# zhengfei0908/SBA-GAN

Hardware: AMD Instinct MI355X
Metric: images/sec (G+D step) at 256px (higher is better)
Workload: dtype bf16; 1 GPU; bird_style.yml 3-stage G+D step (64..256px), B=20 per GPU, G_NET variant=model, image_encoder=inception, text_encoder=RNN_ENCODER in the step; global_batch=20, parallelism=dp1, launch=replayer, losses_finite=True

## Files before the change

include/sbagan_hip.h:

```cpp
#ifndef SBAGAN_HIP_H
#define SBAGAN_HIP_H

#include <stdint.h>

#ifdef __cplusplus
extern "C" {
#endif

#define SBA_F32 0
#define SBA_BF16 1
#define SBA_BF16_YH 2

#define SBA_OK 0
#define SBA_E_ARG (-1)
#define SBA_E_LAUNCH (-2)
#define SBA_E_UNSUPPORTED (-3)

#define SBA_ACT_NONE 0
#define SBA_ACT_GLU 1
#define SBA_ACT_LRELU 2
#define SBA_ACT_RELU 3

#define SBA_MAX_TAPS 32

typedef struct sba_conv_geom {
    int32_t N, IH, IW, Cin;
    int32_t OH, OW, Cout;
    int32_t OHs, OWs;
    int32_t sy, sx;
    int32_t osy, osx, ooy, oox;
    int32_t ups;
    int32_t ntaps;
    int8_t ty[SBA_MAX_TAPS];
    int8_t tx[SBA_MAX_TAPS];
    int32_t x_cstride, x_coff, y_cstride, y_coff;
    int32_t relu;
    int32_t tile, ksplit;
    int32_t first_write;
    int32_t w_layout;
} sba_conv_geom;
#define SBA_IGEMM_TILES 18

const char* sba_version(void);

int sba_set_deterministic(int on, void* scratch, int64_t scratch_bytes);
int sba_get_deterministic(void);
int sba_det_reset(void);
int64_t sba_det_high_water(void);
int sba_set_reduce_scratch(void* scratch, int64_t scratch_bytes);
int sba_bn_stat_slots(void);

int sba_conv_igemm(int dtype, const void* x, const void* w, void* y, const void* addend,
                   float* stats, const sba_conv_geom* g, void* workspace, int64_t workspace_bytes,
                   void* stream);
int sba_conv_igemm_bias(int dtype, const void* x, const void* w, void* y, const void* addend,
                        float* stats, const float* bias, const void* relu_mask, const sba_conv_geom* g,
                        void* workspace, int64_t workspace_bytes, void* stream);
int sba_conv_igemm_plan(int dtype, const sba_conv_geom* g, int64_t workspace_bytes, int* plan);

int sba_fold_bn_pack(int dtype, const float* w, const float* gamma, const float* beta, const float* running_mean,
                     const float* running_var, float eps, void* out, float* bias, int O, int taps, int Cin, int glu,
                     void* stream);
int sba_conv_igemm_glu(int dtype, const void* x, const void* w, const float* bias, void* y, int C,
                       const sba_conv_geom* g, void* stream);
int sba_conv_igemm_glu_plan(int dtype, const sba_conv_geom* g, int C, int* plan);
#define SBA_GROUP_MAX 8
typedef struct sba_conv_group_item {
    const void* x; const void* w; void* y; const void* addend; const float* bias; const void* relu_mask;
    const sba_conv_geom* g;
} sba_conv_group_item;
int sba_conv_igemm_group(int dtype, int n, const sba_conv_group_item* items, int tile, void* stream);
int sba_conv_igemm_group_splitk(int dtype, int n, const sba_conv_group_item* items, int tile, int ksplit,
// ... 216 lines not shown
```

sba-gan_amd/csrc/igemm.hip:

```cpp
#include <math.h>
#include <stdlib.h>

#include "common.h"
#include <type_traits>

namespace {

struct FastDiv {
    uint64_t magic;
    uint32_t d;
};
static inline FastDiv make_fastdiv(uint32_t d, int64_t max_n) {
    FastDiv f;
    f.d = d;
    f.magic = (max_n < (1 << 21) && d > 0) ? (((uint64_t)1 << 42) + d - 1) / d : 0;
    return f;
}
__device__ __forceinline__ uint32_t fdiv(uint32_t n, const FastDiv& f) {
    return f.magic ? (uint32_t)(((uint64_t)n * f.magic) >> 42) : n / f.d;
}

struct EpiX { const float* bias; const void* mask; int yh; int glu_c; };

__device__ __forceinline__ uint32_t relu_mask_bf16x2(uint32_t v, uint32_t m) {
// ... 25 lines not shown
            for (int j = 0; j < TN; ++j)
                b[j] = *reinterpret_cast<const bf16x8_t*>(b_rows + (j * 32 + r) * ROWB + kk * 32 + h * 16);
#pragma unroll
            for (int i = 0; i < TM; ++i)
#pragma unroll
                for (int j = 0; j < TN; ++j)
                    acc[i][j] = __builtin_amdgcn_mfma_f32_32x32x16_bf16(a[i], b[j], acc[i][j], 0, 0, 0);
        }
    }
};

template <> struct Mma<float> {
    template <int TM, int TN, int ROWB>
    static __device__ __forceinline__ void slab(const unsigned char* a_rows, const unsigned char* b_rows,
                                                int lane, f32x16_t (&acc)[TM][TN]) {
        const int r = lane & 31, h = lane >> 5;
#pragma unroll
        for (int kk = 0; kk < 8; ++kk) {
            float a[TM], b[TN];
#pragma unroll
            for (int i = 0; i < TM; ++i)
                a[i] = *reinterpret_cast<const float*>(a_rows + (i * 32 + r) * ROWB + (2 * kk + h) * 4);
#pragma unroll
            for (int j = 0; j < TN; ++j)
                b[j] = *reinterpret_cast<const float*>(b_rows + (j * 32 + r) * ROWB + (2 * kk + h) * 4);
#pragma unroll
            for (int i = 0; i < TM; ++i)
#pragma unroll
                for (int j = 0; j < TN; ++j)
                    acc[i][j] = __builtin_amdgcn_mfma_f32_32x32x2f32(a[i], b[j], acc[i][j], 0, 0, 0);
        }
    }
};

template <typename T, int BM, int BN, int TM, int TN, int NTT, int STAGE_BYTES>
__device__ __forceinline__ void tile_epilogue(f32x16_t (&acc)[TM][TN], const bool lead, unsigned char* lds_all,
                                              const int* rowoff, float* s_stat, const int wm0, const int wn0,
                                              const int lane, const int n_base, const int ycs,
                                              const sba_conv_geom& g, T* __restrict__ y,
                                              const T* __restrict__ addend, float* __restrict__ stats,
                                              const EpiX ex, const int slot_id = -1) {
    const float* __restrict__ bias = ex.bias;
    const T* __restrict__ rmask = reinterpret_cast<const T*>(ex.mask);
    const int col_l = lane & 31, rsel = 4 * (lane >> 5);
    constexpr bool kStageOut = sizeof(T) == 2;
    constexpr int OROW = BN * 2 + 16;
    static_assert(!kStageOut || BM * OROW <= STAGE_BYTES, "output tile fits in the staging buffers");
    if (lead) {
#pragma unroll
    for (int j = 0; j < TN; ++j) {
        const int co = n_base + wn0 + j * 32 + col_l;
        float csum = 0.f, csq = 0.f;
        const float bco = bias ? bias[co < g.Cout ? co : 0] : 0.f;
#pragma unroll
        for (int i = 0; i < TM; ++i) {
#pragma unroll
            for (int r = 0; r < 16; ++r) {
                const int row = wm0 + i * 32 + (r & 3) + 8 * (r >> 2) + rsel;
                float v = acc[i][j][r];
                csum += v;
                csq += v * v;
                if (bias) v += bco;
                if (g.relu) v = fmaxf(v, 0.f);
                if (kStageOut) {
                    *reinterpret_cast<bf16_t*>(lds_all + row * OROW + (wn0 + j * 32 + col_l) * 2) =
                        ex.yh ? f2h_bits(v) : f2bf(v);
                } else {
                    const int pix = rowoff[row];
                    if (pix >= 0 && co < g.Cout) {
                        const int64_t o = (int64_t)pix * ycs + g.y_coff + co;
                        if (addend) v += to_f<T>(addend[o]);
                        if (rmask && !(to_f<T>(rmask[o]) > 0.f)) v = 0.f;
                        y[o] = from_f<T>(v);
                    }
                }
            }
        }
        if (stats) {
            csum += __shfl_xor(csum, 32, 64);
            csq += __shfl_xor(csq, 32, 64);
            if (lane < 32) {
                atomicAdd(&s_stat[wn0 + j * 32 + col_l], csum);
                atomicAdd(&s_stat[BN + wn0 + j * 32 + col_l], csq);
            }
        }
    }
    }
    if (kStageOut || stats) __syncthreads();
    if (kStageOut) {
        constexpr int CPRO = BN / 8;
        for (int idx = threadIdx.x; idx < BM * CPRO; idx += NTT) {
            const int row = idx / CPRO, cc = idx - row * CPRO;
            const int pix = rowoff[row];
            const int co = n_base + cc * 8;
            if (pix < 0 || co >= g.Cout) continue;
            uint4 v = *reinterpret_cast<const uint4*>(lds_all + row * OROW + cc * 16);
            const int64_t o = (int64_t)pix * ycs + g.y_coff + co;
            if (co + 8 <= g.Cout) {
                if (addend) {
                    const uint4 a = *reinterpret_cast<const uint4*>(addend + o);
                    v.x = add_bf16x2(v.x, a.x);
                    v.y = add_bf16x2(v.y, a.y);
                    v.z = add_bf16x2(v.z, a.z);
                    v.w = add_bf16x2(v.w, a.w);
                }
                if (rmask) {
                    const uint4 m = *reinterpret_cast<const uint4*>(rmask + o);
                    v.x = relu_mask_bf16x2(v.x, m.x);
                    v.y = relu_mask_bf16x2(v.y, m.y);
                    v.z = relu_mask_bf16x2(v.z, m.z);
                    v.w = relu_mask_bf16x2(v.w, m.w);
                }
                *reinterpret_cast<uint4*>(y + o) = v;
            } else {
                const uint32_t vw[4] = {v.x, v.y, v.z, v.w};
#pragma unroll
                for (int k = 0; k < 8; ++k) {
                    if (co + k < g.Cout) {
                        float f = bf2f((bf16_t)((k & 1) ? (vw[k >> 1] >> 16) : (vw[k >> 1] & 0xffffu)));
                        if (addend) f += to_f<T>(addend[o + k]);
                        if (rmask && !(to_f<T>(rmask[o + k]) > 0.f)) f = 0.f;
                        y[o + k] = from_f<T>(f);
                    }
                }
            }
        }
    }
    if (stats) {
        const int sid = slot_id >= 0 ? slot_id : (int)(blockIdx.x + blockIdx.z);
        float* slot = stats + (int64_t)(sid & (SBA_BN_STAT_SLOTS - 1)) * 2 * g.Cout;
        for (int c = threadIdx.x; c < BN; c += NTT) {
            const int co = n_base + c;
            if (co < g.Cout) {
                atomicAdd(&slot[co], s_stat[c]);
                atomicAdd(&slot[g.Cout + co], s_stat[BN + c]);
            }
        }
    }
}

template <typename T, int BM, int BN, int TM, int TN, int NTT, int STAGE_BYTES>
__device__ __forceinline__ void tile_epilogue_glu(f32x16_t (&acc)[TM][TN], unsigned char* lds_all, const int* rowoff,
                                                  const int wm0, const int wn0, const int lane, const int n_base,
                                                  const sba_conv_geom& g, T* __restrict__ y, const EpiX ex) {
    static_assert(TN % 2 == 0 && BN % 64 == 0, "a wave owns whole (value, gate) granule pairs");
    const float* __restrict__ bias = ex.bias;
    const int C = ex.glu_c;
    const int ycs = g.y_cstride ? g.y_cstride : C;
    const int col_l = lane & 31, rsel = 4 * (lane >> 5);
    constexpr bool kStageOut = sizeof(T) == 2;
    constexpr int BNO = BN / 2;
    constexpr int OROW = BNO * 2 + 16;
    static_assert(!kStageOut || BM * OROW <= STAGE_BYTES, "output tile fits in the staging buffers");
#pragma unroll
    for (int j = 0; j < TN; j += 2) {
        const int rv = n_base + wn0 + j * 32 + col_l;
        const float bv = bias[rv], bg = bias[rv + 32];
        const int lc = (wn0 >> 1) + (j >> 1) * 32 + col_l;
        const int oc = (n_base >> 1) + lc;
#pragma unroll
        for (int i = 0; i < TM; ++i) {
// ... 2130 lines not shown
            o.y = (uint32_t)f2bf(tile[c8 + 2][r]) | ((uint32_t)f2bf(tile[c8 + 3][r]) << 16);
            o.z = (uint32_t)f2bf(tile[c8 + 4][r]) | ((uint32_t)f2bf(tile[c8 + 5][r]) << 16);
            o.w = (uint32_t)f2bf(tile[c8 + 6][r]) | ((uint32_t)f2bf(tile[c8 + 7][r]) << 16);
            *reinterpret_cast<uint4*>(op) = o;
        } else {
#pragma unroll
            for (int k = 0; k < 8; ++k)
                if (co + k < d.Cout) op[k] = from_f<T>(tile[c8 + k][r]);
        }
    }
}

template <typename T>
__global__ void pool2x2_kernel(const T* __restrict__ up, T* __restrict__ dx, int N, int H, int W, int C) {
    constexpr int V = Vec16<T>::N;
    const int cv = C / V;
    const int64_t total = (int64_t)N * H * W * cv;
    for (int64_t i = blockIdx.x * (int64_t)blockDim.x + threadIdx.x; i < total;
         i += (int64_t)gridDim.x * blockDim.x) {
        const int c = (int)(i % cv) * V;
        int64_t p = i / cv;
        const int xx = (int)(p % W); p /= W;
        const int yy = (int)(p % H);
        const int n = (int)(p / H);
        const T* b = up + (((int64_t)n * 2 * H + 2 * yy) * 2 * W + 2 * xx) * C + c;
        Vec16<T> v00 = ld16(b), v01 = ld16(b + C), v10 = ld16(b + (int64_t)2 * W * C),
                 v11 = ld16(b + (int64_t)2 * W * C + C), o;
#pragma unroll
        for (int k = 0; k < V; ++k) o.set(k, v00.get(k) + v01.get(k) + v10.get(k) + v11.get(k));
        st16(dx + (((int64_t)n * H + yy) * W + xx) * C + c, o);
    }
}

template <typename T>
__device__ __forceinline__ void splitk_finish_body(float* __restrict__ ws, T* __restrict__ y,
                                                   const T* __restrict__ addend,
                                                   float* __restrict__ stats, const sba_conv_geom& g,
                                                   const int M, const EpiX ex) {
    const int ycs = g.y_cstride ? g.y_cstride : g.Cout;
    const int cq = g.Cout / 4;
    const int t = blockIdx.x * blockDim.x + threadIdx.x;
    if (t >= cq) return;
    const int c = t * 4;
    const int m0 = blockIdx.y * 8, m1 = min(m0 + 8, M);
    if (m0 >= M) return;
    const int sub = g.OHs * g.OWs;
    float s0[4] = {0.f, 0.f, 0.f, 0.f}, s1[4] = {0.f, 0.f, 0.f, 0.f};
    float4 rows[8];
#pragma unroll
    for (int r = 0; r < 8; ++r) {
        const int m = m0 + r;
        float4* wp = reinterpret_cast<float4*>(ws + (int64_t)(m < m1 ? m : m0) * g.Cout + c);
        rows[r] = *wp;
        if (m < m1) *wp = make_float4(0.f, 0.f, 0.f, 0.f);
    }
    float bv[4] = {0.f, 0.f, 0.f, 0.f};
    if (ex.bias) {
#pragma unroll
        for (int k = 0; k < 4; ++k) bv[k] = ex.bias[c + k];
    }
#pragma unroll
    for (int r = 0; r < 8; ++r) {
        const int m = m0 + r;
        if (m >= m1) break;
        float v[4] = {rows[r].x, rows[r].y, rows[r].z, rows[r].w};
        const int n = m / sub, rem = m - n * sub;
        const int oy = rem / g.OWs, ox = rem - oy * g.OWs;
        const int64_t o = ((int64_t)(n * g.OH + oy * g.osy + g.ooy) * g.OW + ox * g.osx + g.oox) * ycs + g.y_coff + c;
        typedef typename std::conditional<sizeof(T) == 2, uint2, uint4>::type V4;
        T av[4], mv[4], ov[4];
        if (addend) *reinterpret_cast<V4*>(av) = *reinterpret_cast<const V4*>(addend + o);
        if (ex.mask) *reinterpret_cast<V4*>(mv) = *reinterpret_cast<const V4*>(reinterpret_cast<const T*>(ex.mask) + o);
#pragma unroll
        for (int k = 0; k < 4; ++k) {
            s0[k] += v[k];
            s1[k] += v[k] * v[k];
            v[k] += bv[k];
            if (g.relu) v[k] = fmaxf(v[k], 0.f);
            if (addend) v[k] += to_f<T>(av[k]);
            if (ex.mask && !(to_f<T>(mv[k]) > 0.f)) v[k] = 0.f;
            if (sizeof(T) == 2 && ex.yh) *reinterpret_cast<bf16_t*>(&ov[k]) = f2h_bits(v[k]);
            else ov[k] = from_f<T>(v[k]);
        }
        *reinterpret_cast<V4*>(y + o) = *reinterpret_cast<const V4*>(ov);
    }
    if (stats) {
        float* slot = stats + (int64_t)(blockIdx.y & (SBA_BN_STAT_SLOTS - 1)) * 2 * g.Cout;
#pragma unroll
        for (int k = 0; k < 4; ++k) {
            atomicAdd(&slot[c + k], s0[k]);
            atomicAdd(&slot[g.Cout + c + k], s1[k]);
        }
    }
}

template <typename T>
__global__ __launch_bounds__(256) void splitk_finish_kernel(float* __restrict__ ws, T* __restrict__ y,
                                                            const T* __restrict__ addend,
                                                            float* __restrict__ stats, const sba_conv_geom g,
                                                            const int M, const EpiX ex) {
    splitk_finish_body<T>(ws, y, addend, stats, g, M, ex);
}

__global__ __launch_bounds__(256) void splitk_finish_group_kernel(const GroupArgs A) {
    const GroupItem& it = A.it[blockIdx.z];
    const sba_conv_geom g = it.g;
    splitk_finish_body<bf16_t>(it.ws, it.y, it.addend, nullptr, g, it.M, EpiX{it.bias, it.mask, 0});
}

struct IgemmCfg { int bm, bn, ks, occ; float eff; bool split; };
static const IgemmCfg kCfg[5] = {
    {128, 128, 1, 3, 1.00f, false}, {256, 64, 1, 3, 1.00f, false}, {128, 64, 2, 2, 0.80f, false},
    {64, 64, 2, 4, 0.50f, true},    {320, 128, 2, 1, 0.90f, true}};
constexpr int IGEMM_SPLIT_MAX_M = 2048;

template <typename T, int BM, int BN, int WM, int WN, int KS>
static void launch_cfg(const T* xp, const T* wp, T* yp, const T* ap, float* stats, const sba_conv_geom& g, int M,
                       int nslabs, int split, float* ws, hipStream_t st, const EpiX ex) {
    constexpr int NT = (BM / WM) * (BN / WN) * 64;
    int sps = nslabs;
    if (split > 1) {
        sps = cdiv(cdiv(nslabs, split), KS) * KS;
        split = cdiv(nslabs, sps);
    }
    dim3 grid(cdiv(M, BM), cdiv(g.Cout, BN), split);
    SBA_LAUNCH((igemm_kernel<T, BM, BN, WM, WN, KS>), grid, dim3(NT), 0, st, xp, wp, yp, ap, stats, g, M,
                       split > 1 ? ws : (float*)nullptr, sps, ex);
    if (split > 1) {
        dim3 fgrid(cdiv(g.Cout / 4, 256), cdiv(M, 8));
        SBA_LAUNCH((splitk_finish_kernel<T>), fgrid, dim3(256), 0, st, ws, yp, ap, stats, g, M, ex);
    }
}

static int nmajor_for(const sba_conv_geom& g) {
    const int64_t wb = (int64_t)g.Cout * g.ntaps * g.Cin, xb = (int64_t)g.N * g.IH * g.IW * g.Cin;
    return wb > xb ? 1 : 0;
}

template <int BM, int BN, int WM, int WN, int KS, int D>
static void launch_dma(const bf16_t* xp, const bf16_t* wp, bf16_t* yp, const bf16_t* ap, float* stats,
                       const sba_conv_geom& g, int M, int nslabs, int split, float* ws, hipStream_t st, const EpiX ex) {
    constexpr int NT = (BM / WM) * (BN / WN) * 64;
    int sps = nslabs;
    if (split > 1) {
        sps = cdiv(cdiv(nslabs, split), KS) * KS;
        split = cdiv(nslabs, sps);
    }
    const int gx = cdiv(M, BM), gy = cdiv(g.Cout, BN);
    const int nmajor = nmajor_for(g);
    dim3 grid(nmajor ? 8 * cdiv(gy, 8) * gx : 8 * cdiv(gx, 8) * gy, 1, split);
    SBA_LAUNCH((igemm_dma_kernel<BM, BN, WM, WN, KS, D>), grid, dim3(NT), 0, st, xp, wp, yp, ap, stats, g, M,
               split > 1 ? ws : (float*)nullptr, sps, ex, gx, gy, nmajor DMA_TRACE_ARG);
    if (split > 1) {
        dim3 fgrid(cdiv(g.Cout / 4, 256), cdiv(M, 8));
        SBA_LAUNCH((splitk_finish_kernel<bf16_t>), fgrid, dim3(256), 0, st, ws, yp, ap, stats, g, M, ex);
    }
}

template <int BM, int BN, int WM, int WN, int D>
static void launch_dma2(const bf16_t* xp, const bf16_t* wp, bf16_t* yp, const bf16_t* ap, float* stats,
                        const sba_conv_geom& g, int M, int nslabs64, int split, float* ws, hipStream_t st, const EpiX ex) {
    constexpr int NT = (BM / WM) * (BN / WN) * 64;
    int sps = nslabs64;
    if (split > 1) {
        sps = cdiv(nslabs64, split);
        split = cdiv(nslabs64, sps);
    }
    const int gx = cdiv(M, BM), gy = cdiv(g.Cout, BN);
    const int nmajor = nmajor_for(g);
    dim3 grid(nmajor ? 8 * cdiv(gy, 8) * gx : 8 * cdiv(gx, 8) * gy, 1, split);
    SBA_LAUNCH((igemm_dma2_kernel<BM, BN, WM, WN, D>), grid, dim3(NT), 0, st, xp, wp, yp, ap, stats, g, M,
               split > 1 ? ws : (float*)nullptr, sps, ex, gx, gy, nmajor DMA_TRACE_ARG);
    if (split > 1) {
        dim3 fgrid(cdiv(g.Cout / 4, 256), cdiv(M, 8));
        SBA_LAUNCH((splitk_finish_kernel<bf16_t>), fgrid, dim3(256), 0, st, ws, yp, ap, stats, g, M, ex);
    }
}

static bool halo_ok(const sba_conv_geom& g) {
    if (g.ntaps != 9 || g.sy != 1 || g.sx != 1 || g.osy != 1 || g.osx != 1 || g.ooy || g.oox) return false;
    if (g.OHs != g.OH || g.OWs != g.OW || (g.Cin != 64 && g.Cin != 128) || g.Cout % 64) return false;
    if (g.OH % 8 || g.OW % 32) return false;
    if (g.ups ? (g.IH * 2 != g.OH || g.IW * 2 != g.OW) : (g.IH != g.OH || g.IW != g.OW)) return false;
    for (int t = 0; t < 9; ++t)
        if (g.ty[t] != t / 3 - 1 || g.tx[t] != t % 3 - 1) return false;
    const int64_t tiles = (int64_t)g.N * (g.OH / 8) * (g.OW / 32);
    return tiles >= 128 && tiles <= 0x7fffffff;
}

static bool halo3g_ok(const sba_conv_geom& g) {
    if (g.w_layout != 1 || g.ups) return false;
    if (g.ntaps != 9 || g.sy != 1 || g.sx != 1 || g.osy != 1 || g.osx != 1 || g.ooy || g.oox) return false;
    if (g.OHs != g.OH || g.OWs != g.OW || g.Cin % 32 || g.Cout % 32) return false;
    int ymin = g.ty[0], ymax = g.ty[0], xmin = g.tx[0], xmax = g.tx[0];
    unsigned seen = 0;
    for (int t = 0; t < 9; ++t) {
        ymin = g.ty[t] < ymin ? g.ty[t] : ymin; ymax = g.ty[t] > ymax ? g.ty[t] : ymax;
        xmin = g.tx[t] < xmin ? g.tx[t] : xmin; xmax = g.tx[t] > xmax ? g.tx[t] : xmax;
    }
    if (ymax - ymin != 2 || xmax - xmin != 2) return false;
    for (int t = 0; t < 9; ++t) seen |= 1u << ((g.ty[t] - ymin) * 3 + (g.tx[t] - xmin));
    if (seen != 0x1ffu) return false;
    const int64_t tiles = (int64_t)g.N * cdiv(g.OH, 8) * cdiv(g.OW, 32);
    return tiles >= 128 && tiles <= 0x7fffffff;
}

static void launch_halo3g(const sba_conv_geom& g, const bf16_t* x, const bf16_t* w, bf16_t* y, const bf16_t* addend,
                          const EpiX ex, hipStream_t st) {
    const int tiles = g.N * cdiv(g.OH, 8) * cdiv(g.OW, 32);
    const bool tn2 = g.Cout % 64 == 0;
    dim3 grid(tiles, g.Cout / (tn2 ? 64 : 32));
    if (g.Cin % 64 == 0) {
        if (tn2) SBA_LAUNCH((conv3x3_halo3g_kernel<64, 2>), grid, dim3(256), 0, st, x, w, y, addend, g, ex);
        else SBA_LAUNCH((conv3x3_halo3g_kernel<64, 1>), grid, dim3(256), 0, st, x, w, y, addend, g, ex);
    } else {
        if (tn2) SBA_LAUNCH((conv3x3_halo3g_kernel<32, 2>), grid, dim3(256), 0, st, x, w, y, addend, g, ex);
        else SBA_LAUNCH((conv3x3_halo3g_kernel<32, 1>), grid, dim3(256), 0, st, x, w, y, addend, g, ex);
    }
}

static void launch_halo(const sba_conv_geom& g, const bf16_t* x, const bf16_t* w, bf16_t* y, const bf16_t* addend,
                        float* stats, const EpiX ex, hipStream_t st) {
    const int tiles = g.N * (g.OH / 8) * (g.OW / 32);
    dim3 grid(tiles, g.Cout / 64);
    if (g.w_layout == 1) {
        if (g.ups) SBA_LAUNCH((conv3x3_halo3_kernel<64, 1>), grid, dim3(256), 0, st, x, w, y, addend, stats, g, ex);
        else SBA_LAUNCH((conv3x3_halo3_kernel<64, 0>), grid, dim3(256), 0, st, x, w, y, addend, stats, g, ex);
        return;
    }
    if (g.ups) SBA_LAUNCH((conv3x3_halo_kernel<64, 64, 1>), grid, dim3(256), 0, st, x, w, y, addend, stats, g, ex);
    else SBA_LAUNCH((conv3x3_halo_kernel<64, 64, 0>), grid, dim3(256), 0, st, x, w, y, addend, stats, g, ex);
}

template <typename T>
int launch_igemm(const void* x, const void* w, void* y, const void* addend, float* stats,
                 const sba_conv_geom& g, void* workspace, int64_t ws_bytes, hipStream_t st,
                 const EpiX ex = EpiX{nullptr, nullptr, 0}, int* plan = nullptr) {
    const int M = g.N * g.OHs * g.OWs;
    const T* xp = (const T*)x; const T* wp = (const T*)w; T* yp = (T*)y; const T* ap = (const T*)addend;
    if (g.w_layout != 0 && !(g.w_layout == 1 && sizeof(T) == 2 && (halo_ok(g) || halo3g_ok(g)))) return SBA_E_ARG;
    if (sizeof(T) == 2 && g.w_layout == 1 && !halo_ok(g)) {
        if (plan) { plan[0] = 4; plan[1] = g.Cin % 64 == 0 ? 64 : 32; plan[2] = 1; return SBA_OK; }
        if (stats) return SBA_E_ARG;
        launch_halo3g(g, (const bf16_t*)x, (const bf16_t*)w, (bf16_t*)y, (const bf16_t*)addend, ex, st);
        return SBA_CHECK_LAUNCH();
    }
    if (sizeof(T) == 2 && halo_ok(g)) {
        if (plan) { plan[0] = 0; plan[1] = g.ups ? 1 : 0; plan[2] = 1; return SBA_OK; }
        launch_halo(g, (const bf16_t*)x, (const bf16_t*)w, (bf16_t*)y, (const bf16_t*)addend, stats, ex, st);
        return SBA_CHECK_LAUNCH();
    }
    const int nslabs = g.ntaps * (g.Cin / (64 / (int)sizeof(T)));
    const bool can_split = workspace && g.Cout % 4 == 0 && (int64_t)M * g.Cout * 4 <= ws_bytes && nslabs >= 16;
    int best, best_split = 1;
    const int wgA = (g.Cout % 128 == 0) ? cdiv(M, 128) * (g.Cout / 128) : 0;
    if (M <= 2048) {
        best = (g.Cout >= 1024 && (nslabs >= 512 || (M >= 1280 && nslabs >= 256))) ? 4 : 3;
    } else if ((g.Cout == 128 && M >= 40000) || (g.Cout == 256 && M >= 40000 && nslabs >= 48)) {
        best = 4;
    } else if (wgA >= 320) {
        best = 0;
    } else if (g.Cout <= 64 && cdiv(M, 256) >= 256) {
        best = 1;
    } else if (cdiv(M, 128) * cdiv(g.Cout, 64) >= 256) {
        best = 2;
    } else {
        best = 3;
    }
    {
        const IgemmCfg& k = kCfg[best];
        const int tiles = cdiv(M, k.bm) * cdiv(g.Cout, k.bn);
        const int slots = 256 * k.occ;
        if (k.split && can_split && tiles < slots && M <= IGEMM_SPLIT_MAX_M) {
            int split = slots / tiles;
            if (split > nslabs / 8) split = nslabs / 8;
            if (split > 32) split = 32;
            if (split > 1) best_split = split;
        }
    }
    const bool det = sba_det_on();
// ... 197 lines not shown
    if (O <= 0 || taps <= 0 || Cin <= 0 || (glu && O % 2)) return SBA_E_ARG;
    const int rows = glu ? 64 * ((O / 2 + 31) / 32) : O;
    const int64_t n = (int64_t)rows * taps * Cin;
    if ((int64_t)taps * Cin > 0x7fffffff) return SBA_E_ARG;
    const int blocks = (int)((n + 255) / 256 > 4096 ? 4096 : (n + 255) / 256);
    SBA_DISPATCH(dtype, SBA_LAUNCH((fold_bn_pack_kernel<T>), dim3(blocks), dim3(256), 0, (hipStream_t)stream, w, gamma,
                                   beta, running_mean, running_var, eps, (T*)out, bias, O, taps * Cin, glu, n));
    return SBA_CHECK_LAUNCH();
}

extern "C" int sba_conv_igemm_glu(int dtype, const void* x, const void* w, const float* bias, void* y, int C,
                                  const sba_conv_geom* g, void* stream) {
    sba_conv_geom gg;
    if (!x || !w || !bias || !y || !glu_geom(dtype, g, C, &gg)) return SBA_E_ARG;
    SBA_DISPATCH(dtype, return launch_igemm_glu<T>(x, w, y, gg, (hipStream_t)stream, EpiX{bias, nullptr, 0, C}));
    return SBA_E_ARG;
}

extern "C" int sba_conv_igemm_glu_plan(int dtype, const sba_conv_geom* g, int C, int* plan) {
    sba_conv_geom gg;
    if (!plan || !glu_geom(dtype, g, C, &gg)) return SBA_E_ARG;
    SBA_DISPATCH(dtype, return launch_igemm_glu<T>(nullptr, nullptr, nullptr, gg, nullptr, EpiX{nullptr, nullptr, 0, C}, plan));
    return SBA_E_ARG;
}

extern "C" int sba_conv_igemm(int dtype, const void* x, const void* w, void* y, const void* addend,
                              float* stats, const sba_conv_geom* g, void* workspace, int64_t workspace_bytes,
                              void* stream) {
    if (dtype == SBA_BF16_YH) {
        if (!x || !w || !y || !geom_ok(g, SBA_BF16) || addend || g->relu || g->Cout % 8) return SBA_E_ARG;
        if (((uintptr_t)workspace & 15) != 0) return SBA_E_ARG;
        const EpiX ex{nullptr, nullptr, 1};
        if (sba_det_on() && stats) {
            if (!dense_output(*g)) return SBA_E_ARG;
            const int rc = launch_igemm<bf16_t>(x, w, y, nullptr, nullptr, *g, workspace, workspace_bytes, (hipStream_t)stream, ex);
            if (rc != SBA_OK) return rc;
            return sba_bn_stats(dtype, y, stats, (int64_t)g->N * g->OH * g->OW, 1, g->Cout, stream);
        }
        return launch_igemm<bf16_t>(x, w, y, nullptr, stats, *g, workspace, workspace_bytes, (hipStream_t)stream, ex);
    }
    if (!x || !w || !y || !geom_ok(g, dtype)) return SBA_E_ARG;
    if (((uintptr_t)workspace & 15) != 0) return SBA_E_ARG;
    if (sba_det_on() && stats) {
        if (!dense_output(*g) || addend) return SBA_E_ARG;
        int rc = SBA_E_ARG;
        SBA_DISPATCH(dtype, rc = launch_igemm<T>(x, w, y, addend, nullptr, *g, workspace, workspace_bytes,
                                                 (hipStream_t)stream));
        if (rc != SBA_OK) return rc;
        return sba_bn_stats(dtype, y, stats, (int64_t)g->N * g->OH * g->OW, 1, g->Cout, stream);
    }
    SBA_DISPATCH(dtype, return launch_igemm<T>(x, w, y, addend, stats, *g, workspace, workspace_bytes,
                                               (hipStream_t)stream));
    return SBA_E_ARG;
}

extern "C" int sba_conv_igemm_bias(int dtype, const void* x, const void* w, void* y, const void* addend,
                                   float* stats, const float* bias, const void* relu_mask,
                                   const sba_conv_geom* g, void* workspace, int64_t workspace_bytes, void* stream) {
    if (!x || !w || !y || !geom_ok(g, dtype)) return SBA_E_ARG;
    if (((uintptr_t)workspace & 15) != 0) return SBA_E_ARG;
    if (sba_det_on() && stats) return SBA_E_ARG;
    SBA_DISPATCH(dtype, return launch_igemm<T>(x, w, y, addend, stats, *g, workspace, workspace_bytes,
                                               (hipStream_t)stream, EpiX{bias, relu_mask, 0}));
    return SBA_E_ARG;
}

extern "C" int sba_conv_igemm_plan(int dtype, const sba_conv_geom* g, int64_t workspace_bytes, int* plan) {
    if (!plan || (dtype != SBA_F32 && dtype != SBA_BF16) || !geom_ok(g, dtype)) return SBA_E_ARG;
    static char dummy_ws[16];
    void* ws = workspace_bytes > 0 ? (void*)dummy_ws : nullptr;
    if (dtype == SBA_F32) return launch_igemm<float>(nullptr, nullptr, nullptr, nullptr, nullptr, *g, ws, workspace_bytes,
                                                     nullptr, EpiX{nullptr, nullptr, 0}, plan);
    return launch_igemm<bf16_t>(nullptr, nullptr, nullptr, nullptr, nullptr, *g, ws, workspace_bytes, nullptr,
                                EpiX{nullptr, nullptr, 0}, plan);
}

template <int BM, int BN, int WM, int WN, int D, int KS = 0>
static int launch_group(const sba_conv_group_item* items, int n, hipStream_t st, int split = 1, float* ws = nullptr) {
    GroupArgs A;
    A.n = n;
    A.sps = 0;
    int tiles = 0, max_m = 0, max_co = 0, ns64 = 0;
// ... 307 lines not shown
```

sba-gan_amd/sbagan/_lib.py:

```python
import ctypes
import os

import torch
from ctypes import (POINTER, Structure, byref, c_char_p, c_float, c_int, c_int8, c_int32, c_int64,
                    c_uint64, c_void_p)

_HERE = os.path.dirname(os.path.abspath(__file__))
LIB_PATH = os.environ.get('SBA_LIB_PATH') or os.path.join(os.path.dirname(_HERE), 'csrc', 'libsbagan_hip.so')

SBA_F32, SBA_BF16, SBA_BF16_YH = 0, 1, 2
IGEMM_TILES = 18
ACT_NONE, ACT_GLU, ACT_LRELU, ACT_RELU = 0, 1, 2, 3
MAX_TAPS = 32


class ConvGeom(Structure):
    _fields_ = [('N', c_int32), ('IH', c_int32), ('IW', c_int32), ('Cin', c_int32),
                ('OH', c_int32), ('OW', c_int32), ('Cout', c_int32),
                ('OHs', c_int32), ('OWs', c_int32),
                ('sy', c_int32), ('sx', c_int32),
                ('osy', c_int32), ('osx', c_int32), ('ooy', c_int32), ('oox', c_int32),
                ('ups', c_int32), ('ntaps', c_int32),
                ('ty', c_int8 * MAX_TAPS), ('tx', c_int8 * MAX_TAPS),
                ('x_cstride', c_int32), ('x_coff', c_int32), ('y_cstride', c_int32), ('y_coff', c_int32),
                ('relu', c_int32), ('tile', c_int32), ('ksplit', c_int32), ('first_write', c_int32),
                ('w_layout', c_int32)]


class ConvGroupItem(Structure):
    _fields_ = [('x', c_void_p), ('w', c_void_p), ('y', c_void_p), ('addend', c_void_p), ('bias', c_void_p),
                ('relu_mask', c_void_p), ('g', POINTER(ConvGeom))]


GROUP_MAX = 8

if not os.path.exists(LIB_PATH):
    raise ImportError('libsbagan_hip.so not built: run `python __graft_entry__.py` or '
                      '`make -C sba-gan_amd/csrc` (expected %s)' % LIB_PATH)
lib = ctypes.CDLL(LIB_PATH)

P, I, F, L, U = c_void_p, c_int, c_float, c_int64, c_uint64
G = POINTER(ConvGeom)

SIGNATURES = {
    'sba_conv_igemm': [I, P, P, P, P, P, G, P, L, P],
    'sba_conv_igemm_bias': [I, P, P, P, P, P, P, P, G, P, L, P],
    'sba_conv_igemm_plan': [I, G, L, POINTER(c_int)],
    'sba_fold_bn_pack': [I, P, P, P, P, P, F, P, P, I, I, I, I, P],
    'sba_conv_igemm_glu': [I, P, P, P, P, I, G, P],
    'sba_conv_igemm_glu_plan': [I, G, I, POINTER(c_int)],
    'sba_conv_igemm_group': [I, I, POINTER(ConvGroupItem), I, P],
    'sba_conv_igemm_group_splitk': [I, I, POINTER(ConvGroupItem), I, I, P, L, P],
    'sba_conv_wgrad': [I, P, P, P, G, I, P],
    'sba_pack_weight': [I, P, P, I, I, I, I, I, P],
    'sba_pack_frag_multi': [P, I, I, P],
    'sba_pack_weights_multi': [I, P, I, I, P],
    'sba_pool2x2_sum': [I, P, P, I, I, I, I, P],
    'sba_bn_stats': [I, P, P, L, I, I, P],
    'sba_bn_act_fwd': [I, P, P, P, P, P, P, P, P, P, P, L, I, I, I, I, I, F, F, I, P],
# ... 115 lines not shown
```

sba-gan_amd/sbagan/ops.py:

```python
import ctypes
import os

import torch

from . import _lib
from ._lib import ACT_GLU, ACT_LRELU, ACT_NONE, ConvGeom, call

CL = torch.channels_last
COMPUTE_DTYPE = torch.bfloat16
BN_EPS, BN_MOMENTUM, IN_EPS = 1e-5, 0.1, 1e-5

_WEIGHT_EPOCH = [0]


def set_compute_dtype(dt):
    global COMPUTE_DTYPE
    assert dt in (torch.bfloat16, torch.float32)
    COMPUTE_DTYPE = dt
    _WEIGHT_EPOCH[0] += 1


def compute_dtype():
    return COMPUTE_DTYPE

# ... 386 lines not shown

_TABLE_FILE = None


def _table_section(name):
    global _TABLE_FILE
    if _TABLE_FILE is None:
        _TABLE_FILE = {}
        path = os.environ.get('SBA_IGEMM_TABLE_FILE') or os.path.join(os.path.dirname(os.path.abspath(__file__)),
                                                                      'igemm_table.json')
        if os.environ.get('SBA_IGEMM_TABLE', '1') != '0' and os.path.exists(path):
            import json
            with open(path) as f:
                _TABLE_FILE = json.load(f)
    return _TABLE_FILE.get(name, {})


def _igemm_table():
    global _IGEMM_TABLE
    if _IGEMM_TABLE is None:
        _IGEMM_TABLE = _table_section('bf16')
    return _IGEMM_TABLE


def tune_geom(g, dt):
    if getattr(g, '_tuned', None) != dt:
        g._tuned = dt
        ent = _igemm_table().get(geom_key(g)) if dt == _lib.SBA_BF16 else None
        g.tile, g.ksplit = (int(ent[0]), int(ent[1])) if ent else (0, 0)
    if IGEMM_LOG is not None:
        IGEMM_LOG.append(g)


def _igemm(dt, x, w, y, addend, stats, g, device, w_frag=None):
    ws = workspace(device)
    tune_geom(g, _lib.SBA_BF16 if dt == _lib.SBA_BF16_YH else dt)
    g.w_layout = 0
    if w_frag is not None and _halo_family(g):
        w, g.w_layout = w_frag.data_ptr(), 1
    try:
        call('sba_conv_igemm', dt, x, w, y, addend, stats, ctypes.byref(g), ws.data_ptr(), WORKSPACE_BYTES, _stream())
    finally:
        g.w_layout = 0


def _halo_family(g):
    h = getattr(g, '_halo', None)
    if h is None:
        plan = (ctypes.c_int * 3)()
        old = g.w_layout
        g.w_layout = 0
        call('sba_conv_igemm_plan', _lib.SBA_BF16, ctypes.byref(g), WORKSPACE_BYTES, plan)
        g.w_layout = old
        h = g._halo = plan[0] == 0
    return h




def conv_forward(x, pw, kind, want_stats=True, addend=None, pre_bn=False):
    _need_gpu(x)
    N, Cin, H, W = x.shape
    O = pw.param.shape[0]
    OH, OW = _conv_out_hw(kind, H, W)
    yh = pre_bn and Y_F16 and x.dtype == torch.bfloat16 and addend is None and O % 8 == 0
    if yh:
        y = torch.empty((N, O, OH, OW), dtype=torch.float16, device=x.device, memory_format=CL)
    else:
        y = empty_act(N, O, OH, OW, x)
    stats = zeros_f32((BN_STAT_SLOTS, 2 * O), x.device) if want_stats else None
    g = _geom((kind, N, H, W, Cin, O, None))
    wf = pw.fwd_frag(x.dtype) if kind == '3x3' else None
    _igemm(_lib.SBA_BF16_YH if yh else _dt(x), _p(x), _p(pw.fwd(x.dtype)), _p(y), _p(addend), _p(stats), g, x.device,
           w_frag=wf)
    return y, stats


def conv_dgrad(dy, pw, kind, in_hw, addend=None):
    N, O, OH, OW = dy.shape
    I = pw.param.shape[1]
    H, W = in_hw
    wd = pw.dgrad(dy.dtype, kind)
    if kind == '3x3':
        g = _geom(('3x3', N, OH, OW, O, I, None))
        dx = empty_act(N, I, H, W, dy)
        _igemm(_dt(dy), _p(dy), _p(wd), _p(dx), _p(addend), None, g, dy.device, w_frag=pw.dgrad_frag(dy.dtype, kind))
        return dx
    if kind == '3x3up':
        g = _geom(('4x4s2', N, OH, OW, O, I, None))
        dx = empty_act(N, I, H, W, dy)
        _igemm(_dt(dy), _p(dy), _p(wd), _p(dx), _p(addend), None, g, dy.device)
        return dx
    if kind == '4x4s2':
        dx = empty_act(N, I, H, W, dy)
        esz = dy.element_size()
        gs = [_geom(('4x4s2_dgrad', N, OH, OW, O, I, (cls // 2, cls % 2))) for cls in range(4)]
        if DGRAD4_GROUP and dy.dtype == torch.bfloat16 and O % 64 == 0:
            arr = (_lib.ConvGroupItem * 4)()
            for cls, (a, g) in enumerate(zip(arr, gs)):
                a.x, a.w, a.y, a.addend = _p(dy), wd.data_ptr() + cls * I * 4 * O * esz, _p(dx), _p(addend)
                a.bias = a.relu_mask = None
                a.g = ctypes.pointer(g)
            tile, split = dgrad4_plan(gs[0])
            ws = workspace(dy.device)
            call('sba_conv_igemm_group_splitk', _lib.SBA_BF16, 4, arr, tile, split, ws.data_ptr(), WORKSPACE_BYTES, _stream())
            if IGEMM_LOG is not None:
                IGEMM_LOG.append(('group', tile, gs))
# ... 182 lines not shown
    N, C, H, W = y.shape
    Co = C // 2 if act == ACT_GLU else C
    st = BNState()
    st.C, st.rows, st.groups = C, (N // groups) * H * W, groups
    st.aux = torch.empty((groups, 4, C), dtype=torch.float32, device=y.device)
    out = torch.empty((N, Co, H, W), dtype=_act_dtype(y), device=y.device, memory_format=CL)
    call('sba_bn_act_fwd_fused', _dt(y), _p(y), _p(bn.weight), _p(bn.bias), _p(bn.running_mean), _p(bn.running_var),
         _p(bn.num_batches_tracked), _p(st.aux), _p(out), st.rows, groups, C, act, Co, 0, BN_EPS, BN_MOMENTUM, _stream())
    return out, st


def bn_stats(y, groups=1):
    N, C, H, W = y.shape
    stats = zeros_f32((groups, BN_STAT_SLOTS, 2 * C), y.device)
    call('sba_bn_stats', _dt(y), _p(y), _p(stats), (N // groups) * H * W, groups, C, _stream())
    return stats


def _c(t):
    if t.dim() == 4:
        return t.contiguous(memory_format=CL)
    return t.contiguous()


class ConvBNActFn(torch.autograd.Function):

    @staticmethod
    def forward(ctx, x, weight, gamma, beta, layer, kind, act, residual, groups=1):
        x = as_act(x)
        if groups == 1:
            y, stats = conv_forward(x, layer.pw, kind, want_stats=layer.bn.training, pre_bn=True)
        else:
            assert residual is None and x.shape[0] % groups == 0
            y, _ = conv_forward(x, layer.pw, kind, want_stats=False, pre_bn=True)
            rows_g = (y.shape[0] // groups) * y.shape[2] * y.shape[3]
            if layer.bn.training and rows_g <= BN_FUSED_BWD_ROWS:
                out, sts = bn_act_forward_fused(y, layer.bn, act, groups)
                ctx.layer, ctx.kind, ctx.act, ctx.sts, ctx.groups = layer, kind, act, sts, groups
                ctx.has_res = False
                ctx.save_for_backward(x, y)
                return out
            stats = bn_stats(y, groups) if layer.bn.training else None
        out, sts = bn_act_forward(y, stats, layer.bn, act, residual, groups)
        ctx.layer, ctx.kind, ctx.act, ctx.sts, ctx.groups = layer, kind, act, sts, groups
        ctx.has_res = residual is not None
        ctx.save_for_backward(x, y)
        return out

    @staticmethod
    def backward(ctx, dout):
        x, y = ctx.saved_tensors
        layer, kind, act, groups = ctx.layer, ctx.kind, ctx.act, ctx.groups
        dout = _c(dout)
        dy = bn_act_backward(y, dout, ctx.sts, layer.bn, act, ctx.needs_input_grad[2])
        if ctx.needs_input_grad[1]:
            conv_wgrad_overlapped(x, dy, layer.conv.weight, kind)
        dx = None
        if ctx.needs_input_grad[0]:
            dx = conv_dgrad(dy, layer.pw, kind, x.shape[2:])
        dres = dout if (ctx.has_res and ctx.needs_input_grad[7]) else None
        return dx, None, None, None, None, None, None, dres, None


class ResBlockFn(torch.autograd.Function):

    @staticmethod
    def forward(ctx, x, w1, g1, b1, w2, g2, b2, blk):
        x = as_act(x)
        y1, s1 = conv_forward(x, blk.l1.pw, '3x3', want_stats=blk.l1.bn.training, pre_bn=True)
        a1, st1 = bn_act_forward(y1, s1, blk.l1.bn, ACT_GLU)
        y2, s2 = conv_forward(a1, blk.l2.pw, '3x3', want_stats=blk.l2.bn.training, pre_bn=True)
        out, st2 = bn_act_forward(y2, s2, blk.l2.bn, ACT_NONE, residual=x)
        ctx.blk, ctx.st1, ctx.st2 = blk, st1, st2
        ctx.save_for_backward(x, y1, a1, y2)
        return out
# ... 912 lines not shown
```

Baseline: 2103 images/sec.

## Fuse per-group BatchNorm statistics into the conv igemm epilogue

Adds a stat_rows field so the implicit-GEMM conv epilogue (tile and split-K finish paths) can accumulate BN sum/sumsq per batch group, each group into its own slot array. Grouped ConvBNAct layers then get their statistics from the conv itself instead of a separate bn_stats pass that rereads the output. The cost is extra per-group flush loops with syncthreads and atomics, and grouped calls cannot use the halo 3x3 kernel or the fragment weight layout.

```diff
diff --git a/include/sbagan_hip.h b/include/sbagan_hip.h
--- a/include/sbagan_hip.h
+++ b/include/sbagan_hip.h
@@ -38,6 +38,7 @@
     int32_t tile, ksplit;
     int32_t first_write;
     int32_t w_layout;
+    int32_t stat_rows;
 } sba_conv_geom;
 #define SBA_IGEMM_TILES 18
 
diff --git a/sba-gan_amd/csrc/igemm.hip b/sba-gan_amd/csrc/igemm.hip
--- a/sba-gan_amd/csrc/igemm.hip
+++ b/sba-gan_amd/csrc/igemm.hip
@@ -81,6 +81,54 @@
         }
     }
 };
+
+__device__ __forceinline__ float h_bits2f(bf16_t b) { return (float)__builtin_bit_cast(f16_t, b); }
+
+template <int BN, int NTT>
+__device__ __forceinline__ void group_stats_flush(float* s_stat, float* __restrict__ stats, const int gi, const int sid,
+                                                  const int n_base, const int Cout) {
+    __syncthreads();
+    float* slot = stats + ((int64_t)gi * SBA_BN_STAT_SLOTS + (sid & (SBA_BN_STAT_SLOTS - 1))) * 2 * Cout;
+    for (int c = threadIdx.x; c < BN; c += NTT) {
+        const int co = n_base + c;
+        if (co < Cout) {
+            atomicAdd(&slot[co], s_stat[c]);
+            atomicAdd(&slot[Cout + co], s_stat[BN + c]);
+        }
+        s_stat[c] = 0.f;
+        s_stat[BN + c] = 0.f;
+    }
+    __syncthreads();
+}
+
+template <int BM, int BN, int NTT>
+__device__ __forceinline__ void group_stats_staged(const unsigned char* lds_all, const int* rowoff, float* s_stat,
+                                                   const int n_base, const sba_conv_geom& g,
+                                                   float* __restrict__ stats, const int yh, const int sid) {
+    constexpr int OROW = BN * 2 + 16;
+    static_assert(NTT >= BN, "a thread per staged column");
+    constexpr int RP = NTT / BN;
+    const int p0 = rowoff[0];
+    if (p0 < 0) return;
+    const int nrows = min(BM, g.N * g.OH * g.OW - p0);
+    const int g_lo = p0 / g.stat_rows, g_hi = (p0 + nrows - 1) / g.stat_rows;
+    const int c = (int)threadIdx.x % BN, part = (int)threadIdx.x / BN;
+    for (int gi = g_lo; gi <= g_hi; ++gi) {
+        const int r_lo = max(gi * g.stat_rows - p0, 0), r_hi = min((gi + 1) * g.stat_rows - p0, nrows);
+        if (part < RP) {
+            float s = 0.f, q = 0.f;
+            for (int r = r_lo + part; r < r_hi; r += RP) {
+                const bf16_t b = *reinterpret_cast<const bf16_t*>(lds_all + r * OROW + c * 2);
+                const float v = yh ? h_bits2f(b) : bf2f(b);
+                s += v;
+                q += v * v;
+            }
+            atomicAdd(&s_stat[c], s);
+            atomicAdd(&s_stat[BN + c], q);
+        }
+        group_stats_flush<BN, NTT>(s_stat, stats, gi, sid, n_base, g.Cout);
+    }
+}
 
 template <typename T, int BM, int BN, int TM, int TN, int NTT, int STAGE_BYTES>
 __device__ __forceinline__ void tile_epilogue(f32x16_t (&acc)[TM][TN], const bool lead, unsigned char* lds_all,
@@ -95,6 +143,8 @@
     constexpr bool kStageOut = sizeof(T) == 2;
     constexpr int OROW = BN * 2 + 16;
     static_assert(!kStageOut || BM * OROW <= STAGE_BYTES, "output tile fits in the staging buffers");
+    const bool grouped = stats && g.stat_rows > 0;
+    const bool tstats = stats && !grouped;
     if (lead) {
 #pragma unroll
     for (int j = 0; j < TN; ++j) {
@@ -125,7 +175,7 @@
                 }
             }
         }
-        if (stats) {
+        if (tstats) {
             csum += __shfl_xor(csum, 32, 64);
             csq += __shfl_xor(csq, 32, 64);
             if (lane < 32) {
@@ -175,7 +225,44 @@
             }
         }
     }
-    if (stats) {
+    if (grouped) {
+        const int sid = slot_id >= 0 ? slot_id : (int)(blockIdx.x + blockIdx.z);
+        if constexpr (kStageOut) {
+            group_stats_staged<BM, BN, NTT>(lds_all, rowoff, s_stat, n_base, g, stats, ex.yh, sid);
+        } else {
+            const int p0 = rowoff[0];
+            if (p0 < 0) return;
+            const int p1 = min(p0 + BM, g.N * g.OH * g.OW) - 1;
+            for (int gi = p0 / g.stat_rows; gi <= p1 / g.stat_rows; ++gi) {
+                const int lo = gi * g.stat_rows, hi = lo + g.stat_rows;
+                if (lead) {
+#pragma unroll
+                    for (int j = 0; j < TN; ++j) {
+                        const int co = n_base + wn0 + j * 32 + col_l;
+                        const float bco = bias ? bias[co < g.Cout ? co : 0] : 0.f;
+                        float csum = 0.f, csq = 0.f;
+#pragma unroll
+                        for (int i = 0; i < TM; ++i) {
+#pragma unroll
+                            for (int r = 0; r < 16; ++r) {
+                                const int pix = rowoff[wm0 + i * 32 + (r & 3) + 8 * (r >> 2) + rsel];
+                                float v = acc[i][j][r] + bco;
+                                if (g.relu) v = fmaxf(v, 0.f);
+                                if (pix >= lo && pix < hi) { csum += v; csq += v * v; }
+                            }
+                        }
+                        csum += __shfl_xor(csum, 32, 64);
+                        csq += __shfl_xor(csq, 32, 64);
+                        if (lane < 32) {
+                            atomicAdd(&s_stat[wn0 + j * 32 + col_l], csum);
+                            atomicAdd(&s_stat[BN + wn0 + j * 32 + col_l], csq);
+                        }
+                    }
+                }
+                group_stats_flush<BN, NTT>(s_stat, stats, gi, sid, n_base, g.Cout);
+            }
+        }
+    } else if (stats) {
         const int sid = slot_id >= 0 ? slot_id : (int)(blockIdx.x + blockIdx.z);
         float* slot = stats + (int64_t)(sid & (SBA_BN_STAT_SLOTS - 1)) * 2 * g.Cout;
         for (int c = threadIdx.x; c < BN; c += NTT) {
@@ -2372,7 +2459,7 @@
     }
 }
 
-template <typename T>
+template <typename T, bool GS = false>
 __device__ __forceinline__ void splitk_finish_body(float* __restrict__ ws, T* __restrict__ y,
                                                    const T* __restrict__ addend,
                                                    float* __restrict__ stats, const sba_conv_geom& g,
@@ -2399,10 +2486,27 @@
 #pragma unroll
         for (int k = 0; k < 4; ++k) bv[k] = ex.bias[c + k];
     }
+    const bool grouped = GS && stats && g.stat_rows > 0;
+    int cur_g = grouped ? m0 / g.stat_rows : 0;
+    int g_end = grouped ? (cur_g + 1) * g.stat_rows : 0x7fffffff;
+    auto flush = [&](const int gi) {
+        float* slot = stats + ((int64_t)gi * SBA_BN_STAT_SLOTS + (blockIdx.y & (SBA_BN_STAT_SLOTS - 1))) * 2 * g.Cout;
+#pragma unroll
+        for (int k = 0; k < 4; ++k) {
+            atomicAdd(&slot[c + k], s0[k]);
+            atomicAdd(&slot[g.Cout + c + k], s1[k]);
+            s0[k] = s1[k] = 0.f;
+        }
+    };
 #pragma unroll
     for (int r = 0; r < 8; ++r) {
         const int m = m0 + r;
         if (m >= m1) break;
+        while (GS && m >= g_end) {
+            flush(cur_g);
+            ++cur_g;
+            g_end += g.stat_rows;
+        }
         float v[4] = {rows[r].x, rows[r].y, rows[r].z, rows[r].w};
         const int n = m / sub, rem = m - n * sub;
         const int oy = rem / g.OWs, ox = rem - oy * g.OWs;
@@ -2413,18 +2517,29 @@
         if (ex.mask) *reinterpret_cast<V4*>(mv) = *reinterpret_cast<const V4*>(reinterpret_cast<const T*>(ex.mask) + o);
 #pragma unroll
         for (int k = 0; k < 4; ++k) {
-            s0[k] += v[k];
-            s1[k] += v[k] * v[k];
+            if (!grouped) {
+                s0[k] += v[k];
+                s1[k] += v[k] * v[k];
+            }
             v[k] += bv[k];
             if (g.relu) v[k] = fmaxf(v[k], 0.f);
             if (addend) v[k] += to_f<T>(av[k]);
             if (ex.mask && !(to_f<T>(mv[k]) > 0.f)) v[k] = 0.f;
             if (sizeof(T) == 2 && ex.yh) *reinterpret_cast<bf16_t*>(&ov[k]) = f2h_bits(v[k]);
             else ov[k] = from_f<T>(v[k]);
+            if (grouped) {
+                float sv;
+                if (sizeof(T) == 2 && ex.yh) sv = h_bits2f(*reinterpret_cast<const bf16_t*>(&ov[k]));
+                else sv = to_f<T>(ov[k]);
+                s0[k] += sv;
+                s1[k] += sv * sv;
+            }
         }
         *reinterpret_cast<V4*>(y + o) = *reinterpret_cast<const V4*>(ov);
     }
-    if (stats) {
+    if (grouped) {
+        flush(cur_g);
+    } else if (stats) {
         float* slot = stats + (int64_t)(blockIdx.y & (SBA_BN_STAT_SLOTS - 1)) * 2 * g.Cout;
 #pragma unroll
         for (int k = 0; k < 4; ++k) {
@@ -2434,12 +2549,12 @@
     }
 }
 
-template <typename T>
+template <typename T, bool GS = false>
 __global__ __launch_bounds__(256) void splitk_finish_kernel(float* __restrict__ ws, T* __restrict__ y,
                                                             const T* __restrict__ addend,
                                                             float* __restrict__ stats, const sba_conv_geom g,
                                                             const int M, const EpiX ex) {
-    splitk_finish_body<T>(ws, y, addend, stats, g, M, ex);
+    splitk_finish_body<T, GS>(ws, y, addend, stats, g, M, ex);
 }
 
 __global__ __launch_bounds__(256) void splitk_finish_group_kernel(const GroupArgs A) {
@@ -2453,6 +2568,14 @@
     {128, 128, 1, 3, 1.00f, false}, {256, 64, 1, 3, 1.00f, false}, {128, 64, 2, 2, 0.80f, false},
     {64, 64, 2, 4, 0.50f, true},    {320, 128, 2, 1, 0.90f, true}};
 constexpr int IGEMM_SPLIT_MAX_M = 2048;
+
+template <typename T>
+static void launch_finish(float* ws, T* yp, const T* ap, float* stats, const sba_conv_geom& g, int M, hipStream_t st,
+                          const EpiX ex) {
+    dim3 fgrid(cdiv(g.Cout / 4, 256), cdiv(M, 8));
+    if (stats && g.stat_rows > 0) SBA_LAUNCH((splitk_finish_kernel<T, true>), fgrid, dim3(256), 0, st, ws, yp, ap, stats, g, M, ex);
+    else SBA_LAUNCH((splitk_finish_kernel<T>), fgrid, dim3(256), 0, st, ws, yp, ap, stats, g, M, ex);
+}
 
 template <typename T, int BM, int BN, int WM, int WN, int KS>
 static void launch_cfg(const T* xp, const T* wp, T* yp, const T* ap, float* stats, const sba_conv_geom& g, int M,
@@ -2466,10 +2589,7 @@
     dim3 grid(cdiv(M, BM), cdiv(g.Cout, BN), split);
     SBA_LAUNCH((igemm_kernel<T, BM, BN, WM, WN, KS>), grid, dim3(NT), 0, st, xp, wp, yp, ap, stats, g, M,
                        split > 1 ? ws : (float*)nullptr, sps, ex);
-    if (split > 1) {
-        dim3 fgrid(cdiv(g.Cout / 4, 256), cdiv(M, 8));
-        SBA_LAUNCH((splitk_finish_kernel<T>), fgrid, dim3(256), 0, st, ws, yp, ap, stats, g, M, ex);
-    }
+    if (split > 1) launch_finish<T>(ws, yp, ap, stats, g, M, st, ex);
 }
 
 static int nmajor_for(const sba_conv_geom& g) {
@@ -2491,10 +2611,7 @@
     dim3 grid(nmajor ? 8 * cdiv(gy, 8) * gx : 8 * cdiv(gx, 8) * gy, 1, split);
     SBA_LAUNCH((igemm_dma_kernel<BM, BN, WM, WN, KS, D>), grid, dim3(NT), 0, st, xp, wp, yp, ap, stats, g, M,
                split > 1 ? ws : (float*)nullptr, sps, ex, gx, gy, nmajor DMA_TRACE_ARG);
-    if (split > 1) {
-        dim3 fgrid(cdiv(g.Cout / 4, 256), cdiv(M, 8));
-        SBA_LAUNCH((splitk_finish_kernel<bf16_t>), fgrid, dim3(256), 0, st, ws, yp, ap, stats, g, M, ex);
-    }
+    if (split > 1) launch_finish<bf16_t>(ws, yp, ap, stats, g, M, st, ex);
 }
 
 template <int BM, int BN, int WM, int WN, int D>
@@ -2511,10 +2628,7 @@
     dim3 grid(nmajor ? 8 * cdiv(gy, 8) * gx : 8 * cdiv(gx, 8) * gy, 1, split);
     SBA_LAUNCH((igemm_dma2_kernel<BM, BN, WM, WN, D>), grid, dim3(NT), 0, st, xp, wp, yp, ap, stats, g, M,
                split > 1 ? ws : (float*)nullptr, sps, ex, gx, gy, nmajor DMA_TRACE_ARG);
-    if (split > 1) {
-        dim3 fgrid(cdiv(g.Cout / 4, 256), cdiv(M, 8));
-        SBA_LAUNCH((splitk_finish_kernel<bf16_t>), fgrid, dim3(256), 0, st, ws, yp, ap, stats, g, M, ex);
-    }
+    if (split > 1) launch_finish<bf16_t>(ws, yp, ap, stats, g, M, st, ex);
 }
 
 static bool halo_ok(const sba_conv_geom& g) {
@@ -2572,12 +2686,21 @@
     else SBA_LAUNCH((conv3x3_halo_kernel<64, 64, 0>), grid, dim3(256), 0, st, x, w, y, addend, stats, g, ex);
 }
 
+bool dense_output(const sba_conv_geom& g);
+static bool group_stats_ok(const sba_conv_geom& g, const void* addend, const EpiX& ex) {
+    if (g.stat_rows < 0 || !dense_output(g) || addend || ex.mask || ex.glu_c) return false;
+    const int64_t hw = (int64_t)g.OH * g.OW, rows = (int64_t)g.N * hw;
+    if (g.stat_rows % hw || rows % g.stat_rows) return false;
+    return g.w_layout == 0;
+}
+
 template <typename T>
 int launch_igemm(const void* x, const void* w, void* y, const void* addend, float* stats,
                  const sba_conv_geom& g, void* workspace, int64_t ws_bytes, hipStream_t st,
                  const EpiX ex = EpiX{nullptr, nullptr, 0}, int* plan = nullptr) {
     const int M = g.N * g.OHs * g.OWs;
     const T* xp = (const T*)x; const T* wp = (const T*)w; T* yp = (T*)y; const T* ap = (const T*)addend;
+    if (stats && g.stat_rows && !plan && !group_stats_ok(g, addend, ex)) return SBA_E_ARG;
     if (g.w_layout != 0 && !(g.w_layout == 1 && sizeof(T) == 2 && (halo_ok(g) || halo3g_ok(g)))) return SBA_E_ARG;
     if (sizeof(T) == 2 && g.w_layout == 1 && !halo_ok(g)) {
         if (plan) { plan[0] = 4; plan[1] = g.Cin % 64 == 0 ? 64 : 32; plan[2] = 1; return SBA_OK; }
@@ -2585,7 +2708,7 @@
         launch_halo3g(g, (const bf16_t*)x, (const bf16_t*)w, (bf16_t*)y, (const bf16_t*)addend, ex, st);
         return SBA_CHECK_LAUNCH();
     }
-    if (sizeof(T) == 2 && halo_ok(g)) {
+    if (sizeof(T) == 2 && halo_ok(g) && !(stats && g.stat_rows)) {
         if (plan) { plan[0] = 0; plan[1] = g.ups ? 1 : 0; plan[2] = 1; return SBA_OK; }
         launch_halo(g, (const bf16_t*)x, (const bf16_t*)w, (bf16_t*)y, (const bf16_t*)addend, stats, ex, st);
         return SBA_CHECK_LAUNCH();
@@ -2849,10 +2972,11 @@
         if (((uintptr_t)workspace & 15) != 0) return SBA_E_ARG;
         const EpiX ex{nullptr, nullptr, 1};
         if (sba_det_on() && stats) {
-            if (!dense_output(*g)) return SBA_E_ARG;
+            if (!dense_output(*g) || (g->stat_rows && !group_stats_ok(*g, nullptr, ex))) return SBA_E_ARG;
             const int rc = launch_igemm<bf16_t>(x, w, y, nullptr, nullptr, *g, workspace, workspace_bytes, (hipStream_t)stream, ex);
             if (rc != SBA_OK) return rc;
-            return sba_bn_stats(dtype, y, stats, (int64_t)g->N * g->OH * g->OW, 1, g->Cout, stream);
+            const int64_t rows = (int64_t)g->N * g->OH * g->OW, rpg = g->stat_rows ? g->stat_rows : rows;
+            return sba_bn_stats(dtype, y, stats, rpg, (int)(rows / rpg), g->Cout, stream);
         }
         return launch_igemm<bf16_t>(x, w, y, nullptr, stats, *g, workspace, workspace_bytes, (hipStream_t)stream, ex);
     }
@@ -2860,11 +2984,13 @@
     if (((uintptr_t)workspace & 15) != 0) return SBA_E_ARG;
     if (sba_det_on() && stats) {
         if (!dense_output(*g) || addend) return SBA_E_ARG;
+        if (g->stat_rows && !group_stats_ok(*g, addend, EpiX{nullptr, nullptr, 0})) return SBA_E_ARG;
         int rc = SBA_E_ARG;
         SBA_DISPATCH(dtype, rc = launch_igemm<T>(x, w, y, addend, nullptr, *g, workspace, workspace_bytes,
                                                  (hipStream_t)stream));
         if (rc != SBA_OK) return rc;
-        return sba_bn_stats(dtype, y, stats, (int64_t)g->N * g->OH * g->OW, 1, g->Cout, stream);
+        const int64_t rows = (int64_t)g->N * g->OH * g->OW, rpg = g->stat_rows ? g->stat_rows : rows;
+        return sba_bn_stats(dtype, y, stats, rpg, (int)(rows / rpg), g->Cout, stream);
     }
     SBA_DISPATCH(dtype, return launch_igemm<T>(x, w, y, addend, stats, *g, workspace, workspace_bytes,
                                                (hipStream_t)stream));
diff --git a/sba-gan_amd/sbagan/_lib.py b/sba-gan_amd/sbagan/_lib.py
--- a/sba-gan_amd/sbagan/_lib.py
+++ b/sba-gan_amd/sbagan/_lib.py
@@ -24,7 +24,7 @@
                 ('ty', c_int8 * MAX_TAPS), ('tx', c_int8 * MAX_TAPS),
                 ('x_cstride', c_int32), ('x_coff', c_int32), ('y_cstride', c_int32), ('y_coff', c_int32),
                 ('relu', c_int32), ('tile', c_int32), ('ksplit', c_int32), ('first_write', c_int32),
-                ('w_layout', c_int32)]
+                ('w_layout', c_int32), ('stat_rows', c_int32)]
 
 
 class ConvGroupItem(Structure):
diff --git a/sba-gan_amd/sbagan/ops.py b/sba-gan_amd/sbagan/ops.py
--- a/sba-gan_amd/sbagan/ops.py
+++ b/sba-gan_amd/sbagan/ops.py
@@ -442,16 +442,17 @@
         IGEMM_LOG.append(g)
 
 
-def _igemm(dt, x, w, y, addend, stats, g, device, w_frag=None):
+def _igemm(dt, x, w, y, addend, stats, g, device, w_frag=None, stat_rows=0):
     ws = workspace(device)
     tune_geom(g, _lib.SBA_BF16 if dt == _lib.SBA_BF16_YH else dt)
     g.w_layout = 0
-    if w_frag is not None and _halo_family(g):
+    if w_frag is not None and stat_rows == 0 and _halo_family(g):
         w, g.w_layout = w_frag.data_ptr(), 1
+    g.stat_rows = stat_rows
     try:
         call('sba_conv_igemm', dt, x, w, y, addend, stats, ctypes.byref(g), ws.data_ptr(), WORKSPACE_BYTES, _stream())
     finally:
-        g.w_layout = 0
+        g.w_layout = g.stat_rows = 0
 
 
 def _halo_family(g):
@@ -468,7 +469,7 @@
 
 
 
-def conv_forward(x, pw, kind, want_stats=True, addend=None, pre_bn=False):
+def conv_forward(x, pw, kind, want_stats=True, addend=None, pre_bn=False, groups=1):
     _need_gpu(x)
     N, Cin, H, W = x.shape
     O = pw.param.shape[0]
@@ -478,11 +479,16 @@
         y = torch.empty((N, O, OH, OW), dtype=torch.float16, device=x.device, memory_format=CL)
     else:
         y = empty_act(N, O, OH, OW, x)
-    stats = zeros_f32((BN_STAT_SLOTS, 2 * O), x.device) if want_stats else None
+    stat_rows = 0
+    if want_stats and groups > 1:
+        assert N % groups == 0 and addend is None
+        stats, stat_rows = zeros_f32((groups, BN_STAT_SLOTS, 2 * O), x.device), (N // groups) * OH * OW
+    else:
+        stats = zeros_f32((BN_STAT_SLOTS, 2 * O), x.device) if want_stats else None
     g = _geom((kind, N, H, W, Cin, O, None))
     wf = pw.fwd_frag(x.dtype) if kind == '3x3' else None
     _igemm(_lib.SBA_BF16_YH if yh else _dt(x), _p(x), _p(pw.fwd(x.dtype)), _p(y), _p(addend), _p(stats), g, x.device,
-           w_frag=wf)
+           w_frag=wf, stat_rows=stat_rows)
     return y, stats
 
 
@@ -731,15 +737,16 @@
             y, stats = conv_forward(x, layer.pw, kind, want_stats=layer.bn.training, pre_bn=True)
         else:
             assert residual is None and x.shape[0] % groups == 0
-            y, _ = conv_forward(x, layer.pw, kind, want_stats=False, pre_bn=True)
-            rows_g = (y.shape[0] // groups) * y.shape[2] * y.shape[3]
+            OH, OW = _conv_out_hw(kind, x.shape[2], x.shape[3])
+            rows_g = (x.shape[0] // groups) * OH * OW
             if layer.bn.training and rows_g <= BN_FUSED_BWD_ROWS:
+                y, _ = conv_forward(x, layer.pw, kind, want_stats=False, pre_bn=True)
                 out, sts = bn_act_forward_fused(y, layer.bn, act, groups)
                 ctx.layer, ctx.kind, ctx.act, ctx.sts, ctx.groups = layer, kind, act, sts, groups
                 ctx.has_res = False
                 ctx.save_for_backward(x, y)
                 return out
-            stats = bn_stats(y, groups) if layer.bn.training else None
+            y, stats = conv_forward(x, layer.pw, kind, want_stats=layer.bn.training, pre_bn=True, groups=groups)
         out, sts = bn_act_forward(y, stats, layer.bn, act, residual, groups)
         ctx.layer, ctx.kind, ctx.act, ctx.sts, ctx.groups = layer, kind, act, sts, groups
         ctx.has_res = residual is not None
```

After: 2118 images/sec (median of 6 runs). No clear change (+0.7%).
